# HKUST-Aerial-Robotics/Omni-swarm

Measured on AMD Instinct MI355X. Metric: keyframes/sec (4x fisheye 600x480) + p50 loop-match ms @ 100k-frame DB, higher is better.
Workload: dtype f16

## Files before the change

### omni-swarm_amd/csrc/config.h

```cpp
#pragma once
#include "common.h"

namespace omni {

enum CfgId {
    CFG_CONV_V1 = 0, CFG_RS_TRN, CFG_DET16, CFG_SP_SPARSE_DESC, CFG_SP_SPARSE_DA, CFG_SP_FUSED_CAND, CFG_SP_SPLIT_DB, CFG_SP_MASK_SKIP, CFG_SP_MASK_SKIP_SPLIT, CFG_SPLIT_FUSE1A, CFG_SPLIT_WINO,
    CFG_SPLIT_TRN, CFG_CONV_XCD, CFG_SP_PROFILE_MASK, CFG_PP_U8, CFG_PP_TRACE, CFG_PP_DBG, CFG_RS_TRACE, CFG_SPLIT_TRACE, CFG_SPLIT_DBG, CFG_WINO_TRACE, CFG_ROCTX,
    CFG_VLAD_BIG, CFG_VLAD_STEM_FUSE, CFG_VLAD_UNFUSED, CFG_VLAD_MFMA, CFG_VLAD_SBLOCK, CFG_VLAD_MBLOCK_PX, CFG_VLAD_MFMA_PX, CFG_VLAD_FC_MFMA, CFG_VLAD_MBLOCK_CPW,
    CFG_VLAD_SB_LDSPAD, CFG_VLAD_SB_PERSIST, CFG_VLAD_SB_TRACE, CFG_VLAD_SB_DBG, CFG_VLAD_MASK_SKIP,
    CFG_SCAN_ROWS_MIN, CFG_MQ_ROT, CFG_MQ_MIN, CFG_INDEX_MIRROR, CFG_INDEX_MIRROR_MIN_ROWS, CFG_INDEX_CERT_FAIL,
    CFG_GEOMETRY_THREADS, CFG_MESSAGE_THREADS, CFG_GEOMETRY_ASYNC, CFG_DETECTOR_ASYNC, CFG_PIPELINE_ONE_STREAM, CFG_PIPELINE_FIFO, CFG_PIPELINE_UNIT_PLAN,
    CFG_HW_QUEUES,
    CFG_RCCL_LIB,
    CFG_COUNT
};
enum CfgClass {
    CFG_VARIANT = 0,
    CFG_TUNING = 1,
    CFG_DEBUG = 2,
    CFG_TEST = 3,
    CFG_STRING = 4
};
struct CfgOption { const char* env; int def, lo, hi; int cls; const char* doc; };
extern const CfgOption kCfgOptions[CFG_COUNT];

struct Config {
    int v[CFG_COUNT];
    int operator[](CfgId i) const { return v[i]; }
};
int config_resolve(Config* out);
const Config& config_process();
int config_option_now(CfgId i);

}
```

### omni-swarm_amd/csrc/config.hip

```cpp
#include "config.h"

#include <atomic>
#include <cerrno>
#include <climits>
#include <cstdlib>

namespace omni {

const CfgOption kCfgOptions[CFG_COUNT] = {
    {"OMNI_CONV_V1", 0, 0, 3, CFG_VARIANT, "fp16 3x3 layers: 0 = production (conv1a fused into the ping-pong conv1b, register-stationary cin=128); 1 = generic kernel, 2 = persistent LDS-DMA kernel, "
                                           "3 = ping-pong without the conv1a fusion -- 1-3 exist only in the test build of the library (lib_test/)"},
    {"OMNI_RS_TRN", -1, -1, 1, CFG_VARIANT, "register-stationary kernel of the unpooled cin=128 fp16 layers: tile orientation, -1 = the one with fewer tiles, 0 = plain, 1 = transposed"},
    {"OMNI_DET16", 1, 0, 1, CFG_VARIANT, "detector head of the fp16 and OMNI_PREC_SPLIT paths on v_mfma_f32_32x32x16_f16 with split (hi, lo) operands (0: the exact-f32 MFMA kernel)"},
    {"OMNI_SP_SPARSE_DESC", 1, 0, 1, CFG_VARIANT, "convDb + descriptor norm only at the cells around the key points (0: dense descriptor map)"},
    {"OMNI_SP_SPARSE_DA", 1, 0, 1, CFG_VARIANT, "convDa only at those cells too (fp16 and OMNI_PREC_SPLIT; 0: dense convDa)"},
    {"OMNI_SP_FUSED_CAND", 1, 0, 1, CFG_VARIANT, "getKeyPoints' threshold inside the detector head's epilogue + window masks from the candidate list (0: sp_cand_kernel re-reads the heat map)"},
    {"OMNI_SP_SPLIT_DB", 1, 0, 1, CFG_VARIANT, "OMNI_PREC_SPLIT: convDb + descriptor norm at the key points' cells with split (hi, lo) operands on the fp16 matrix cores (0: exact-f32 MFMA convolution)"},
    {"OMNI_SP_MASK_SKIP", 1, 0, 1, CFG_VARIANT, "fp16: the tiles inside the constant region of the fisheye mask are left out of the tile walk (0: every tile)"},
    {"OMNI_SP_MASK_SKIP_SPLIT", 1, 0, 1, CFG_VARIANT, "the same for OMNI_PREC_SPLIT"},
    {"OMNI_SPLIT_FUSE1A", 1, 0, 1, CFG_VARIANT, "OMNI_PREC_SPLIT: conv1a built inside the conv1b kernel from the u8 image (0: separate exact-f32 conv1a pass)"},
    {"OMNI_SPLIT_WINO", 7, 0, 15, CFG_VARIANT, "OMNI_PREC_SPLIT: the cin = 64 layers as Winograd F(2x2,3x3) kernels with split operands (conv_wino.hip), bit 0 = conv1b (with the conv1a "
                                                "fusion), 1 = conv2a, 2 = conv2b, 3 = conv3a (off by default: same time as the direct kernel, profiles/r06g); 0: the direct kernels of conv_split.hip"},
    {"OMNI_SPLIT_TRN", -1, -1, 1, CFG_VARIANT, "OMNI_PREC_SPLIT cin=128 kernel: tile orientation, as OMNI_RS_TRN"},
    {"OMNI_CONV_XCD", 1, 0, 1, CFG_VARIANT, "persistent convolution kernels derive (cout group, tile walk) from an XCD-aware block id: the cout groups of a pixel tile and its neighbours "
                                           "share one L2 (0: plain blockIdx; process-wide, same results either way)"},
    {"OMNI_SP_PROFILE_MASK", 0, 0, 1, CFG_TUNING, "omni_sp_profile times the stages with the fisheye mask on (what the key-frame pipeline runs)"},
    {"OMNI_PP_U8", 1, 0, 1, CFG_VARIANT, "fp16 conv1a inside conv1b's kernel: matrix-core operands straight from the image bytes (0: through the 256-entry u8 -> (hi, lo) table in LDS)"},
    {"OMNI_PP_TRACE", 0, 0, 1, CFG_DEBUG, "s_memtime trace of the ping-pong conv kernel on stderr"},
    {"OMNI_PP_DBG", 0, 0, 255, CFG_DEBUG, "ping-pong conv kernel timing ablations (WRONG results)"},
    {"OMNI_RS_TRACE", 0, 0, 1, CFG_DEBUG, "s_memtime trace of the register-stationary kernel"},
    {"OMNI_SPLIT_TRACE", 0, 0, 1, CFG_DEBUG, "s_memtime trace of the split-precision kernel"},
    {"OMNI_SPLIT_DBG", 0, 0, 3, CFG_DEBUG, "split-precision kernel timing ablations: 1 = no stores, 2 = every DMA reads tile 0 (WRONG results)"},
    {"OMNI_WINO_TRACE", 0, 0, 1, CFG_DEBUG, "s_memtime trace of the Winograd split kernel"},
    {"OMNI_ROCTX", 0, 0, 1, CFG_DEBUG, "roctx ranges around upload / SuperPoint / MobileNetVLAD / post-processing / BF match / index add + search / exchange and the host loop's "
                                      "stages (rocprofv3 --marker-trace; the library is resolved by dlopen)"},
    {"OMNI_VLAD_BIG", 0, 0, 128, CFG_TUNING, "64 / 128: the 64- / 128-pixel tiles of the unfused block kernel (measured slower at 600x480)"},
    {"OMNI_VLAD_STEM_FUSE", 1, 0, 1, CFG_VARIANT, "stem + block 0 in one kernel (0: two kernels)"},
    {"OMNI_VLAD_UNFUSED", 0, 0, 1, CFG_VARIANT, "1: every block as expand / depthwise / project launches"},
    {"OMNI_VLAD_MFMA", 1, 0, 1, CFG_VARIANT, "late blocks' 1x1 convolutions on the matrix cores"},
    {"OMNI_VLAD_SBLOCK", 1, 0, 1, CFG_VARIANT, "fused split-fp16 block kernel (vlad_s.hip)"},
    {"OMNI_VLAD_MBLOCK_PX", 2048, 0, 1 << 24, CFG_TUNING, "fused matrix-core block kernel for blocks of at most this many input pixels per image (0 disables)"},
    {"OMNI_VLAD_MFMA_PX", 0, 0, 1 << 24, CFG_TUNING, "> 0: matrix-core 1x1 convolutions for blocks of at most this many input pixels per image (default 2048)"},
    {"OMNI_VLAD_FC_MFMA", 1, 0, 1, CFG_VARIANT, "the final FC on the matrix cores (0: VALU kernel)"},
    {"OMNI_VLAD_MBLOCK_CPW", 0, 0, 64, CFG_TUNING, "hidden-layer split of the matrix-core block kernel: chunks per workgroup (0 = no split; measured: does not pay)"},
    {"OMNI_VLAD_SB_LDSPAD", 0, 0, 160 * 1024, CFG_DEBUG, "extra LDS bytes per workgroup of the split block kernel (occupancy A/B)"},
    {"OMNI_VLAD_SB_PERSIST", 1, 0, 16, CFG_VARIANT, "split block kernel: 0 = one tile per workgroup, N >= 1 = N x (CUs x resident workgroups) persistent workgroups"},
    {"OMNI_VLAD_SB_TRACE", 0, 0, 1, CFG_DEBUG, "s_memtime trace of the split block kernel"},
    {"OMNI_VLAD_SB_DBG", 0, 0, 255, CFG_DEBUG, "split block kernel timing ablations (WRONG results)"},
    {"OMNI_VLAD_MASK_SKIP", 1, 0, 1, CFG_VARIANT, "fisheye-masked passes leave the tiles of the first blocks that lie in the constant region of the mask out of the tile walk "
                                                  "(bit-identical; 0: the dense pass)"},
    {"OMNI_SCAN_ROWS_MIN", 4, 1, 1 << 20, CFG_TUNING, "fp32 scan: from this many queries on, the rows-stationary kernel"},
    {"OMNI_MQ_ROT", 1, 0, 1, CFG_VARIANT, "matrix-core multi-query scan: rotated query fragments"},
    {"OMNI_MQ_MIN", 4, 0, 1 << 20, CFG_TUNING, "queries from which an fp16 shard is searched on the matrix cores (1 = always, 0 = never)"},
    {"OMNI_INDEX_MIRROR", 1, 0, 1, CFG_VARIANT, "fp32 index: fp16 mirror + certificate for batched searches (0: exact scans only)"},
    {"OMNI_INDEX_MIRROR_MIN_ROWS", 32768, 0, INT_MAX, CFG_TUNING, "the mirror is used from this many rows on"},
    {"OMNI_INDEX_CERT_FAIL", 0, 0, 1, CFG_TEST, "1: every certificate fails (exercises the exact fallback)"},
    {"OMNI_GEOMETRY_THREADS", -1, -1, 1024, CFG_TUNING, "threads of the geometric-verification pool (-1: min(16, cores / 2); 0: inline)"},
    {"OMNI_MESSAGE_THREADS", 3, 0, 64, CFG_TUNING, "helper threads that fill a unit's key-frame messages (key points, descriptors, lifted points: ~75 KB per image, first-touch page "
                                                  "faults included) next to the calling thread while the unit's detector step runs on the GPU (0: inline)"},
    {"OMNI_GEOMETRY_ASYNC", 1, 0, 1, CFG_VARIANT, "a micro-batch's geometry tasks run while the next unit is waited for (0: drained at once)"},
    {"OMNI_DETECTOR_ASYNC", 1, 0, 1, CFG_VARIANT, "a micro-batch's detector step (appends, searches) is enqueued and collected one unit later (0: the host waits for it on the spot)"},
    {"OMNI_PIPELINE_ONE_STREAM", 0, 0, 1, CFG_VARIANT, "a unit's MobileNetVLAD launches behind its SuperPoint launches on one stream (0: next to them on a second stream)"},
    {"OMNI_PIPELINE_FIFO", -1, -1, 2, CFG_VARIANT, "units in flight run oldest first: a unit's SuperPoint stream (1) / both its streams (2) start behind the convolution stack of the unit "
                                                   "enqueued before it; 0: the units' kernels take turns; -1: by measurement -- 1 for the fp32-class precisions, whose time is all "
                                                   "CU-filling convolutions (+2-4 %), and for an fp16 run() of no more units than lanes (all in flight at once: +13 % at 3 units), 0 for fp16 otherwise, whose small-grid "
                                                   "tails the next units' kernels fill (-5 % when chained)"},
    {"OMNI_PIPELINE_UNIT_PLAN", 1, 0, 2, CFG_VARIANT, "KeyframePipeline::run on host blocks, a run that is not a whole number of micro-batches: 1 = units of equal size (20 key frames = "
                                                       "7 + 7 + 6), 2 = the same behind half a unit, 0 = the blocks' own cut (8 + 8 + 4)"},
    {"OMNI_HW_QUEUES", 8, 0, 64, CFG_TUNING, "hardware queues asked of the HIP runtime when the library is loaded (GPU_MAX_HW_QUEUES, unless already set): the pipeline's five "
                                            "streams must not share one; 0 = the runtime's default of 4"},
    {"OMNI_RCCL_LIB", 0, 0, 0, CFG_STRING, "path of the RCCL library omni_shard dlopens (default: librccl.so next to torch, then the loader's search path)"},
};

static int parse_one(const CfgOption& o, int* out, bool* bad) {
    *out = o.def; *bad = false;
    if (o.cls == CFG_STRING) return 0;
    const char* e = getenv(o.env);
    if (!e || !e[0]) return 0;
    errno = 0;
    char* end = nullptr;
    const long v = strtol(e, &end, 10);
    if (errno || end == e || *end != '\0' || v < o.lo || v > o.hi) { *bad = true; return 0; }
    *out = (int)v;
    return 1;
}

int config_resolve(Config* out) {
    for (int i = 0; i < CFG_COUNT; ++i) {
        bool bad;
        parse_one(kCfgOptions[i], &out->v[i], &bad);
        OMNI_REQUIRE(!bad, OMNI_ERR_INVALID, "%s=%s: expected an integer in [%d, %d] (%s)", kCfgOptions[i].env, getenv(kCfgOptions[i].env), kCfgOptions[i].lo, kCfgOptions[i].hi,
                     kCfgOptions[i].doc);
    }
    return OMNI_OK;
}

static bool is_process_wide(int i) {
    switch (i) {
        case CFG_CONV_XCD: case CFG_INDEX_CERT_FAIL: case CFG_INDEX_MIRROR: case CFG_INDEX_MIRROR_MIN_ROWS: case CFG_MQ_ROT:
        case CFG_PP_DBG: case CFG_PP_TRACE: case CFG_RS_TRACE: case CFG_RS_TRN: case CFG_SCAN_ROWS_MIN: case CFG_SPLIT_DBG: case CFG_SPLIT_TRACE: case CFG_SPLIT_TRN: case CFG_WINO_TRACE: case CFG_ROCTX:
        case CFG_VLAD_BIG: case CFG_VLAD_SB_DBG: case CFG_VLAD_SB_LDSPAD: case CFG_VLAD_SB_TRACE:
            return true;
        default:
            return false;
    }
}
static std::atomic<bool> g_process_resolved{false};

int config_option_now(CfgId i) {
    int v; bool bad;
    parse_one(kCfgOptions[i], &v, &bad);
    return v;
}

const Config& config_process() {
    static const Config c = [] {
        g_process_resolved.store(true);
        Config q;
        for (int i = 0; i < CFG_COUNT; ++i) {
            bool bad;
            parse_one(kCfgOptions[i], &q.v[i], &bad);
            if (bad) fprintf(stderr, "libomni_hip: %s=%s ignored: expected an integer in [%d, %d]\n", kCfgOptions[i].env, getenv(kCfgOptions[i].env), kCfgOptions[i].lo, kCfgOptions[i].hi);
        }
        return q;
    }();
    return c;
}

}

extern "C" {

int omni_config_count(void) { return omni::CFG_COUNT; }
// ... 31 lines not shown
```

### omni-swarm_amd/csrc/vlad.hip

```cpp
#include "config.h"
#include "common.h"
#include "vlad_h.h"
#include "conv.h"

struct VladLayerDev { int kind, cin, cout, stride, hin, win, hout, wout; float* w; float* b; };

struct VladFusedBlock {
    int cin, hid, cout, stride, expand, res, hin, win, hout, wout;
    const float* bp;
    float* blob;
    float* mblob;
    void* hblob;
    void* sblob;
    int cop;
    const float *we_t, *be, *wd_t, *bd, *wp_t;
};

struct omni_vlad {
    omni_ctx* ctx = nullptr;
    omni::Config cfg;
    bool sblock = true;
    int prec = OMNI_PREC_F32;
    bool fused = false;
    bool mfma_late = true;
    int mblock_max_px = 0;
    int mfma_max_px = 2048;
    std::vector<VladFusedBlock> blocks;
    int W = 0, H = 0, max_batch = 0, K = 0, Dm = 0, out_dim = 0, hf = 0, wf = 0;
    std::vector<VladLayerDev> layers;
    float *assign_wT = nullptr, *assign_b = nullptr, *clusters = nullptr, *fc_w = nullptr, *fc_b = nullptr;
    float* mb_partial = nullptr; size_t mb_partial_bytes = 0; int mb_cpw = 1;
    float *fc_wp = nullptr, *fc_part = nullptr;
    bool fc_mfma = false;
    float *buf[3] = {nullptr, nullptr, nullptr};
    size_t buf_elems = 0;
    float *assign = nullptr, *vlad = nullptr, *out = nullptr;
    uint8_t* gray_stage = nullptr;
    omni::HostBuf hstage;
    struct MaskSkip {
        int ty0 = 0, ty1 = 0, tx0 = 0, tx1 = 0;
        int oy0 = 0, oy1 = 0, ox0 = 0, ox1 = 0;
        int oh = 0, ow = 0, oc = 0;
        float* buf = nullptr;
        void* vec = nullptr;
        double frac = 0.0;
    };
    std::vector<MaskSkip> mskip;
    bool mask_skip_ready = false;
    uint8_t* zero_gray = nullptr;
    std::mutex mu;
};

namespace omni {

__device__ __forceinline__ float relu6f(float v) { return fminf(fmaxf(v, 0.f), 6.f); }

__global__ void __launch_bounds__(256)
vlad_stem_kernel(const uint8_t* __restrict__ gray, int stride, int H, int W, int mask0, int mask1, int Ho, int Wo, int cout,
                 int cstride, const float* __restrict__ w , const float* __restrict__ bias, float* __restrict__ out) {
    const int b = blockIdx.y;
    const int p = blockIdx.x * 256 + threadIdx.x;
    if (p >= Ho * Wo) return;
    const int oy = p / Wo, ox = p - oy * Wo;
    const uint8_t* g = gray + (int64_t)b * stride * H;
    float v[9];
#pragma unroll
    for (int t = 0; t < 9; ++t) {
        const int y = oy * cstride - 1 + t / 3, x = ox * cstride - 1 + t % 3;
        float px = 0.f;
        if (y >= 0 && y < H && x >= 0 && x < W) {
            const float raw = (y >= mask0 && y < mask1) ? 0.f : (float)g[(int64_t)y * stride + x];
            px = (raw - 128.0f) / 128.0f;
        }
        v[t] = px;
    }
    float* o = out + ((int64_t)b * Ho * Wo + p) * cout;
    for (int c = 0; c < cout; ++c) {
        float acc = bias[c];
#pragma unroll
        for (int t = 0; t < 9; ++t) acc = fmaf(v[t], w[c * 9 + t], acc);
        o[c] = relu6f(acc);
    }
}

__global__ void __launch_bounds__(256)
// ... 880 lines not shown
    __shared__ float patch[PH * PW];
    __shared__ __attribute__((aligned(16))) float h[R * 16];
    __shared__ __attribute__((aligned(16))) float d[SB_TW * SB_TH * 16];
    __shared__ float s_ws[16 * 9], s_bs[16], s_wd[9 * 16], s_bd[16];
    const int tid = threadIdx.x, b = blockIdx.y;
    const int tiles_x = (Wo + SB_TW - 1) / SB_TW;
    const int oy0 = (blockIdx.x / tiles_x) * SB_TH, ox0 = (blockIdx.x % tiles_x) * SB_TW;
    const int sy0 = oy0 - 1, sx0 = ox0 - 1;
    const int iy0 = 2 * sy0 - 1, ix0 = 2 * sx0 - 1;
    if (tid < 144) { s_ws[tid] = ws[tid]; s_wd[tid] = wd_t[tid]; }
    if (tid < 16) { s_bs[tid] = bs[tid]; s_bd[tid] = bd[tid]; }
    const uint8_t* g = gray + (int64_t)b * stride * H;
    for (int i = tid; i < PH * PW; i += 256) {
        const int y = iy0 + i / PW, x = ix0 + i % PW;
        float px = 0.f;
        if (y >= 0 && y < H && x >= 0 && x < W) {
            const float raw = (y >= mask0 && y < mask1) ? 0.f : (float)g[(int64_t)y * stride + x];
            px = (raw - 128.0f) / 128.0f;
        }
        patch[i] = px;
    }
    __syncthreads();
    for (int i = tid; i < R * 4; i += 256) {
        const int r = i >> 2, c4 = (i & 3) * 4;
        const int ry = r / RW, rx = r - ry * RW;
        const int sy = sy0 + ry, sx = sx0 + rx;
        float4 res = make_float4(0.f, 0.f, 0.f, 0.f);
        if (sy >= 0 && sy < Ho && sx >= 0 && sx < Wo) {
            float v[9];
#pragma unroll
            for (int t = 0; t < 9; ++t) v[t] = patch[(2 * ry + t / 3) * PW + 2 * rx + t % 3];
            float rr[4];
#pragma unroll
            for (int j = 0; j < 4; ++j) {
                float acc = s_bs[c4 + j];
#pragma unroll
                for (int t = 0; t < 9; ++t) acc = fmaf(v[t], s_ws[(c4 + j) * 9 + t], acc);
                rr[j] = relu6f(acc);
            }
            res = make_float4(rr[0], rr[1], rr[2], rr[3]);
        }
        *reinterpret_cast<float4*>(h + r * 16 + c4) = res;
    }
    __syncthreads();
    for (int i = tid; i < SB_TW * SB_TH * 4; i += 256) {
        const int o = i >> 2, c4 = (i & 3) * 4;
        const int oy = o / SB_TW, ox = o - oy * SB_TW;
        float t[4];
#pragma unroll
        for (int j = 0; j < 4; ++j) t[j] = s_bd[c4 + j];
#pragma unroll
        for (int dy = 0; dy < 3; ++dy)
#pragma unroll
            for (int dx = 0; dx < 3; ++dx) {
                const float4 x = *reinterpret_cast<const float4*>(h + ((oy + dy) * RW + ox + dx) * 16 + c4);
                const float* wv = s_wd + (dy * 3 + dx) * 16 + c4;
                t[0] = fmaf(x.x, wv[0], t[0]); t[1] = fmaf(x.y, wv[1], t[1]); t[2] = fmaf(x.z, wv[2], t[2]); t[3] = fmaf(x.w, wv[3], t[3]);
            }
        *reinterpret_cast<float4*>(d + o * 16 + c4) = make_float4(relu6f(t[0]), relu6f(t[1]), relu6f(t[2]), relu6f(t[3]));
    }
    __syncthreads();
    {
        const int co = tid & 7, og = tid >> 3;
        float wp[16];
#pragma unroll
        for (int k = 0; k < 16; ++k) wp[k] = wp_t[k * 8 + co];
        const float bpv = bp[co];
#pragma unroll
        for (int i = 0; i < 4; ++i) {
            const int o = og + 32 * i;
            float acc = 0.f;
#pragma unroll
            for (int k4 = 0; k4 < 4; ++k4) {
                const float4 x = *reinterpret_cast<const float4*>(d + o * 16 + k4 * 4);
                acc = fmaf(x.x, wp[k4 * 4 + 0], acc); acc = fmaf(x.y, wp[k4 * 4 + 1], acc);
                acc = fmaf(x.z, wp[k4 * 4 + 2], acc); acc = fmaf(x.w, wp[k4 * 4 + 3], acc);
            }
            const int oy = oy0 + o / SB_TW, ox = ox0 + o % SB_TW;
            if (oy < Ho && ox < Wo) out[(((int64_t)b * Ho + oy) * Wo + ox) * 8 + co] = acc + bpv;
        }
    }
}

static int vlad_backbone_fused(omni_vlad* v, const uint8_t* gray_dev, int stride, int batch, int fisheye_mask, int skip_mode, const float** out_ptr) {
    hipStream_t st = v->ctx->stream;
    const int H = v->H, W = v->W;
    const float* in_over = nullptr;
    int m0, m1;
    omni_fisheye_mask_rows(H, fisheye_mask, &m0, &m1);
    const VladLayerDev& S = v->layers[0];
    int cur = 0, rc;
    size_t first = 0;
    const bool stem_fuse = v->cfg[omni::CFG_VLAD_STEM_FUSE] != 0;
    const VladFusedBlock* B0 = v->blocks.empty() ? nullptr : &v->blocks[0];
    if (stem_fuse && B0 && S.cout == 16 && S.stride == 2 && !B0->expand && !B0->res && B0->cin == 16 && B0->hid == 16 && B0->cout == 8 &&
        B0->stride == 1) {
        hipLaunchKernelGGL(vlad_stem_b0_kernel, dim3(cdiv(B0->wout, SB_TW) * cdiv(B0->hout, SB_TH), batch), dim3(256), 0, st, gray_dev, stride, H,
                           W, m0, m1, S.hout, S.wout, S.w, S.b, B0->wd_t, B0->bd, B0->wp_t, B0->bp, skip_mode ? v->mskip[0].buf : v->buf[1],
                           skip_mode == 2 ? v->mskip[0].ty0 : 0, skip_mode == 2 ? v->mskip[0].ty1 : 0, v->mskip.empty() ? 0 : v->mskip[0].tx0, v->mskip.empty() ? 0 : v->mskip[0].tx1);
        OMNI_LAUNCH_CHECK();
        cur = 1; first = 1;
        if (skip_mode) in_over = v->mskip[0].buf;
    } else {
        hipLaunchKernelGGL(vlad_stem4_kernel, dim3(cdiv(S.hout * S.wout * (S.cout / 4), 256), batch), dim3(256), 0, st, gray_dev, stride, H, W, m0,
                           m1, S.hout, S.wout, S.cout, S.stride, S.w, S.b, v->buf[0]);
        OMNI_LAUNCH_CHECK();
    }
    for (size_t bi = first; bi < v->blocks.size(); ++bi) {
        const VladFusedBlock& B = v->blocks[bi];
        const int64_t Pin = (int64_t)batch * B.hin * B.win, Pout = (int64_t)batch * B.hout * B.wout;
        const float* const in = in_over ? in_over : v->buf[cur];
        in_over = nullptr;
        if (v->prec == OMNI_PREC_F16 && B.hblob) {
            VladHBlockArgs ha;
            ha.in = in; ha.out = v->buf[(cur + 1) % 3]; ha.blob = B.hblob; ha.bp = B.bp;
            ha.Hi = B.hin; ha.Wi = B.win; ha.Ho = B.hout; ha.Wo = B.wout; ha.cin = B.cin; ha.hid = B.hid; ha.cout = B.cout; ha.res = B.res; ha.batch = batch;
            if ((rc = launch_vlad_hblock(st, ha, B.stride))) return rc;
            cur = (cur + 1) % 3;
            continue;
        }
        if (v->sblock && B.sblob) {
            VladSBlockArgs sa;
            const bool own = skip_mode && bi < v->mskip.size();
            sa.in = in; sa.out = own ? v->mskip[bi].buf : v->buf[(cur + 1) % 3]; sa.blob = B.sblob; sa.bp = B.bp;
            if (own && skip_mode == 2) { sa.sk_y0 = v->mskip[bi].ty0; sa.sk_y1 = v->mskip[bi].ty1; sa.sk_x0 = v->mskip[bi].tx0; sa.sk_w = v->mskip[bi].tx1 - v->mskip[bi].tx0; }
            sa.Hi = B.hin; sa.Wi = B.win; sa.Ho = B.hout; sa.Wo = B.wout; sa.cin = B.cin; sa.hid = B.hid; sa.cout = B.cout; sa.res = B.res; sa.batch = batch;
            sa.n_cu = v->ctx->prop.multiProcessorCount > 0 ? v->ctx->prop.multiProcessorCount : 256; sa.trace = nullptr; sa.dbg = 0;
            sa.persist = v->cfg[omni::CFG_VLAD_SB_PERSIST];
            if ((rc = launch_vlad_sblock(st, sa, B.stride))) return rc;
            if (own) in_over = v->mskip[bi].buf;
            else cur = (cur + 1) % 3;
            continue;
        }
        if (B.mblob && B.hin * B.win <= v->mblock_max_px) {
            VladMBlockArgs m;
            m.in = in; m.out = v->buf[(cur + 1) % 3]; m.blob = B.mblob; m.bp = B.bp;
            m.Hi = B.hin; m.Wi = B.win; m.Ho = B.hout; m.Wo = B.wout; m.cin = B.cin; m.hid = B.hid; m.cout = B.cout; m.cop = B.cop;
            m.stride = B.stride; m.res = B.res; m.batch = batch;
            const int n_chunks = (B.hid + 31) / 32, tiles = cdiv(B.wout, 8) * cdiv(B.hout, 8) * batch;
            m.cpw = v->mb_cpw > 0 ? v->mb_cpw : n_chunks; m.n_groups = cdiv(n_chunks, m.cpw);
            if ((size_t)tiles * m.n_groups * 64 * B.cop * 4 > v->mb_partial_bytes) { m.cpw = n_chunks; m.n_groups = 1; }
            m.partial = v->mb_partial;
            if ((rc = launch_vlad_mblock(st, m))) return rc;
            cur = (cur + 1) % 3;
            continue;
        }
        if (B.expand && B.cin % 8 == 0 && B.hid % 8 == 0 && B.hin * B.win <= v->mfma_max_px && v->mfma_late) {
            const int e = (cur + 1) % 3, d = (cur + 2) % 3;
            if ((rc = vlad_pw_mfma(st, in, Pin, B.cin, B.hid, B.we_t, B.be, nullptr, 1, v->buf[e]))) return rc;
            const int64_t total = Pout * (B.hid / 4);
            hipLaunchKernelGGL(vlad_dw_kernel, dim3((unsigned)cdiv64(total, 256)), dim3(256), 0, st, v->buf[e], B.hin, B.win, B.hid, B.hout, B.wout,
                               B.stride, B.wd_t, B.bd, v->buf[d], total);
            OMNI_LAUNCH_CHECK();
            if ((rc = vlad_pw_mfma(st, v->buf[d], Pout, B.hid, B.cout, B.wp_t, B.bp, B.res ? in : nullptr, 0, v->buf[e]))) return rc;
            cur = e;
            continue;
        }
        VladBlockArgs a;
        a.in = in; a.out = v->buf[(cur + 1) % 3];
        a.blob = B.blob; a.bp = B.bp;
        a.Hi = B.hin; a.Wi = B.win; a.Ho = B.hout; a.Wo = B.wout; a.hid = B.hid; a.cout = B.cout; a.stride = B.stride;
        a.expand = B.expand; a.res = B.res; a.batch = batch;
        if ((rc = vlad_block(st, B.cin, a))) return rc;
        cur = (cur + 1) % 3;
    }
    *out_ptr = in_over ? in_over : v->buf[cur];
    return OMNI_OK;
}

static int vlad_calibrate_mask_skip(omni_vlad* v) {
    hipStream_t st = v->ctx->stream;
    if (!v->zero_gray) {
        OMNI_HIP_TRY(hipMalloc((void**)&v->zero_gray, (size_t)v->W * v->H));
        OMNI_HIP_TRY(hipMemsetAsync(v->zero_gray, 0, (size_t)v->W * v->H, st));
    }
    const float* unused;
    int rc;
    if ((rc = vlad_backbone_fused(v, v->zero_gray, v->W, 1, 1, 1, &unused))) return rc;
    for (const omni_vlad::MaskSkip& k : v->mskip) {
        const int pix = k.oc * 4;
        const int64_t row = (int64_t)k.ow * pix, img = row * k.oh;
        if ((rc = conv_read_pixel_bytes(st, k.buf, row, 0, pix, (k.oy0 + k.oy1) / 2, (k.ox0 + k.ox1) / 2, k.vec))) return rc;
        if ((rc = conv_fill_rect_bytes(st, k.buf, v->max_batch, img, row, 0, pix, k.oy0, k.oy1, k.ox0, k.ox1, k.vec))) return rc;
// ... 372 lines not shown
```

### omni-swarm_amd/csrc/vlad_s.hip

```cpp
#include "config.h"
#include "common.h"
#include "vlad_h.h"

namespace omni {

typedef _Float16 sh8 __attribute__((ext_vector_type(8)));
typedef _Float16 sh4 __attribute__((ext_vector_type(4)));
typedef _Float16 sh2 __attribute__((ext_vector_type(2)));
typedef float sf16 __attribute__((ext_vector_type(16)));
typedef float sf2 __attribute__((ext_vector_type(2)));
typedef float sf4 __attribute__((ext_vector_type(4)));

#define SB_CH 48
#define SB_HS 208
#define SB_DS 112
#define SB_WD (10 * SB_CH)

__device__ __forceinline__ int sb_div(int n, unsigned m) { return m ? (int)__umulhi((unsigned)n, m) : n; }

template <int STRIDE, int CIN, int NT>
struct SBlockCfg {
    static constexpr int S1 = (2 * CIN + 2 + 15) / 16, S2 = (CIN + 15) / 16;
    static constexpr int XS = S1 * 32 + 16;
    static constexpr int TH = STRIDE == 1 ? 8 : 4, OPX = 8 * TH, NTN = OPX / 32;
// ... 7 lines not shown
#ifndef SB_WPE_SMALL
#define SB_WPE_SMALL 2
#endif
template <int STRIDE, int CIN, int NT>
__global__ void __launch_bounds__((SBlockCfg<STRIDE, CIN, NT>::THREADS), (CIN > 32 ? 1 : (CIN <= 16 ? SB_WPE_SMALL : 2)))
vlad_sblock_kernel(VladSBlockArgs a) {
    using C = SBlockCfg<STRIDE, CIN, NT>;
    constexpr int S1 = C::S1, S2 = C::S2, XS = C::XS, TH = C::TH, OPX = C::OPX, RWX = C::RWX, R = C::R, CB = C::CB, MQ = C::MQ, NW = C::NW, RT = C::RT, XP = C::XP;
    extern __shared__ __attribute__((aligned(16))) char smem[];
    const int n_chunks = a.hid / SB_CH;
    char* xin = smem;
    char* dhi = smem + R * XS;
    char* dlo = dhi + OPX * SB_DS;
    char* h = dlo + OPX * SB_DS;
    float* wdl = reinterpret_cast<float*>(h + R * SB_HS);
    const int tid = threadIdx.x, lane = tid & 63, wave = __builtin_amdgcn_readfirstlane(tid >> 6);
    const int n = lane & 31, kk = lane >> 5;
    const int tiles_x = (a.Wo + 7) >> 3, tiles_y = (a.Ho + TH - 1) / TH, tiles_img = tiles_x * tiles_y;
    const char* blob = reinterpret_cast<const char*>(a.blob);
    const char* frag = blob + (size_t)n_chunks * SB_WD * 4;

    sh8 we1[S1][2], we2[S2][2];
    auto load_we = [&](int c) {
        const char* cb = frag + (int64_t)c * CB + lane * 16;
#pragma unroll
        for (int ks = 0; ks < S1; ++ks)
#pragma unroll
            for (int m = 0; m < 2; ++m) we1[ks][m] = *reinterpret_cast<const sh8*>(cb + (ks * 2 + m) * 1024);
#pragma unroll
        for (int ks = 0; ks < S2; ++ks)
#pragma unroll
            for (int m = 0; m < 2; ++m) we2[ks][m] = *reinterpret_cast<const sh8*>(cb + ((S1 + ks) * 2 + m) * 1024);
    };
    load_we(0);
    {
        const sf4* ws = reinterpret_cast<const sf4*>(blob);
        for (int e = tid; e < n_chunks * (SB_WD / 4); e += C::THREADS) reinterpret_cast<sf4*>(wdl)[e] = ws[e];
    }
    const int pair = tid % 24, blk = tid / 24;
    const int nt = STRIDE == 1 ? (wave & 1) : 0;
    const int mt0 = STRIDE == 1 ? (wave >> 1) : wave;
    constexpr int MSTEP = STRIDE == 1 ? 2 : NW;
    const bool pwave = mt0 < NT;
    sf4 pbias[MQ][4];
#pragma unroll
    for (int q = 0; q < MQ; ++q)
#pragma unroll
        for (int g = 0; g < 4; ++g) {
            const int ch = (mt0 + MSTEP * q) * 32 + 8 * g + 4 * kk;
            const sf4 z = {0.f, 0.f, 0.f, 0.f};
            pbias[q][g] = ch < a.cout ? *reinterpret_cast<const sf4*>(a.bp + ch) : z;
        }

    auto tile_origin = [&](int tile, int& tb, int& toy, int& tox) {
        tb = sb_div(tile, a.m_img);
        const int ttr = tile - tb * tiles_img, tty = sb_div(ttr, a.m_tx);
        toy = tty * TH; tox = (ttr - tty * tiles_x) * 8;
    };
    const int act_total = a.walk.act * a.batch;
    auto full_tile = [&](int t) -> int {
        if (a.walk.y1 <= a.walk.y0) return t;
        const int tb = sb_div(t, a.m_act);
        return tb * tiles_img + tile_walk_index(a.walk, tiles_x, t - tb * a.walk.act);
    };
    const int xhf = tid & 1;
    sf4 xpre[XP][CIN / 8];
    bool xin_img[XP];
    auto fetch_x = [&](int tile) {
        int tb, toy, tox;
        tile_origin(tile, tb, toy, tox);
#pragma unroll
        for (int ps = 0; ps < XP; ++ps) {
            const int xr = (tid >> 1) + ps * (C::THREADS / 2), xry = xr / RWX, xrx = xr - xry * RWX;
            const int gy = toy * STRIDE - 1 + xry, gx = tox * STRIDE - 1 + xrx;
            xin_img[ps] = xr < R && gy >= 0 && gy < a.Hi && gx >= 0 && gx < a.Wi;
            const unsigned off = (unsigned)((tb * a.Hi + gy) * a.Wi + gx) * CIN + xhf * (CIN / 2);
#pragma unroll
            for (int q = 0; q < CIN / 8; ++q) {
                const sf4 z = {0.f, 0.f, 0.f, 0.f};
                xpre[ps][q] = xin_img[ps] ? *reinterpret_cast<const sf4*>(a.in + off + q * 4) : z;
            }
        }
    };
    sf16 acc[MQ];
    sf4 resv[MQ][4];
    unsigned out_off = 0;
    bool out_ok = false;
    auto out_pixel = [&](int tile, unsigned& off_out, unsigned& off_res) {
        int tb, toy, tox;
        tile_origin(tile, tb, toy, tox);
        const int o = nt * 32 + n, oy = toy + (o >> 3), ox = tox + (o & 7);
        off_out = (unsigned)((tb * a.Ho + oy) * a.Wo + ox) * (unsigned)a.cout;
        off_res = (unsigned)((tb * a.Hi + oy) * a.Wi + ox) * (unsigned)CIN;
        return pwave && oy < a.Ho && ox < a.Wo;
    };
    auto fetch_res = [&](bool ok, unsigned off_res) {
        if (!a.res) return;
#pragma unroll
        for (int q = 0; q < MQ; ++q)
#pragma unroll
            for (int g = 0; g < 4; ++g) {
                const int ch = (mt0 + MSTEP * q) * 32 + 8 * g + 4 * kk;
                const sf4 z = {0.f, 0.f, 0.f, 0.f};
                resv[q][g] = (ok && ch < a.cout) ? *reinterpret_cast<const sf4*>(a.in + off_res + ch) : z;
            }
    };
    auto store_out = [&]() {
        if (!out_ok || (a.dbg & 1)) return;
#pragma unroll
        for (int q = 0; q < MQ; ++q)
#pragma unroll
            for (int g = 0; g < 4; ++g) {
                const int ch = (mt0 + MSTEP * q) * 32 + 8 * g + 4 * kk;
                if (ch >= a.cout) continue;
                sf4 v = pbias[q][g];
#pragma unroll
                for (int j = 0; j < 4; ++j) v[j] += acc[q][4 * g + j];
                if (a.res) v += resv[q][g];
                *reinterpret_cast<sf4*>(a.out + out_off + ch) = v;
            }
    };

    auto expand = [&]() {
#pragma unroll
      for (int rt = 0; rt < (RT + NW - 1) / NW; ++rt) {
        const int rw = wave + rt * NW;
        if (rw >= RT) break;
        const char* xb = xin + (rw * 32 + n) * XS + kk * 16;
        sf16 e0, e1;
#pragma unroll
        for (int r = 0; r < 16; ++r) { e0[r] = 0.f; e1[r] = 0.f; }
#pragma unroll
        for (int ks = 0; ks < S1; ++ks) {
            const sh8 xb8 = *reinterpret_cast<const sh8*>(xb + ks * 32);
            e0 = __builtin_amdgcn_mfma_f32_32x32x16_f16(we1[ks][0], xb8, e0, 0, 0, 0);
            e1 = __builtin_amdgcn_mfma_f32_32x32x16_f16(we1[ks][1], xb8, e1, 0, 0, 0);
        }
#pragma unroll
        for (int ks = 0; ks < S2; ++ks) {
            const sh8 xb8 = *reinterpret_cast<const sh8*>(xb + ks * 32);
            e0 = __builtin_amdgcn_mfma_f32_32x32x16_f16(we2[ks][0], xb8, e0, 0, 0, 0);
            e1 = __builtin_amdgcn_mfma_f32_32x32x16_f16(we2[ks][1], xb8, e1, 0, 0, 0);
        }
        if (rw * 32 + n < R) {
            char* hp = h + (rw * 32 + n) * SB_HS + kk * 16;
#pragma unroll
            for (int g = 0; g < 4; ++g) {
                sf4 v;
#pragma unroll
                for (int j = 0; j < 4; ++j) v[j] = __builtin_amdgcn_fmed3f(e0[4 * g + j], 0.f, 6.f);
                *reinterpret_cast<sf4*>(hp + g * 32) = v;
            }
#pragma unroll
            for (int g = 0; g < 2; ++g) {
                sf4 v;
#pragma unroll
                for (int j = 0; j < 4; ++j) v[j] = __builtin_amdgcn_fmed3f(e1[4 * g + j], 0.f, 6.f);
                *reinterpret_cast<sf4*>(hp + 128 + g * 32) = v;
            }
        }
      }
    };

    if ((int)blockIdx.x < act_total) fetch_x(full_tile(blockIdx.x));
#define TR(k) do { if (trw) a.trace[wave * 16 + (k)] = __builtin_amdgcn_s_memtime(); } while (0)
    for (int t = blockIdx.x; t < act_total; t += gridDim.x) {
        const int tile = full_tile(t);
        const bool trw = a.trace && blockIdx.x == 0 && (tid & 63) == 0 && t == (int)blockIdx.x + 2 * (int)gridDim.x;
        TR(8);
#pragma unroll
        for (int ps = 0; ps < XP; ++ps) {
            const int xr = (tid >> 1) + ps * (C::THREADS / 2);
            if (xr < R) {
                char* row = xin + xr * XS;
#pragma unroll
                for (int q = 0; q < CIN / 8; ++q) {
                    const sf4 v = xpre[ps][q];
                    const sh4 hi = __builtin_convertvector(v, sh4);
                    const sh4 lo = __builtin_convertvector(v - __builtin_convertvector(hi, sf4), sh4);
                    *reinterpret_cast<sh4*>(row + (xhf * (CIN / 2) + q * 4) * 2) = hi;
                    *reinterpret_cast<sh4*>(row + CIN * 2 + (xhf * (CIN / 2) + q * 4) * 2) = lo;
                }
                sh8 t = {0, 0, 0, 0, 0, 0, 0, 0};
                if (xhf == 0 && xin_img[ps]) { t[0] = (_Float16)1.f; t[1] = (_Float16)1.f; }
                *reinterpret_cast<sh8*>(row + CIN * 4 + xhf * 16) = t;
            }
        }
        store_out();
        {
            unsigned off_res;
            out_ok = out_pixel(tile, out_off, off_res);
            fetch_res(out_ok, off_res);
        }
        if (t + (int)gridDim.x < act_total && !(a.dbg & 2)) fetch_x(full_tile(t + gridDim.x));
#pragma unroll
        for (int p = 0; p < MQ; ++p)
#pragma unroll
            for (int r = 0; r < 16; ++r) acc[p][r] = 0.f;

        __syncthreads();
        TR(0);
// ... 76 lines not shown
                expand();
                __syncthreads();
            }
            TR(6);
        }
        TR(7);
    }
#undef TR
    store_out();
}

static inline uint16_t sb_f2h(float v) { const __half hv = __float2half_rn(v); uint16_t u; memcpy(&u, &hv, 2); return u; }
static inline float sb_h2f(uint16_t u) { __half hv; memcpy(&hv, &u, 2); return __half2float(hv); }
static inline float sb_hi(float v) { return sb_h2f(sb_f2h(v)); }
static inline float sb_lo(float v) { return v - sb_hi(v); }

#define SB_SHAPES(X) X(2, 8, 1) X(1, 8, 1) X(1, 16, 1) X(2, 16, 1) X(1, 24, 1) X(1, 32, 1) X(2, 32, 2) X(1, 56, 2) X(1, 56, 4)

bool vlad_sblock_supported(int cin, int hid, int cout, int stride) {
    if (hid < SB_CH || hid % SB_CH || cout % 4 || cout < 4) return false;
    const int nt0 = (cout + 31) / 32, nt = nt0 == 3 ? 4 : nt0;
#define X(S, CI, N) if (stride == S && cin == CI && nt == N) return true;
    SB_SHAPES(X)
#undef X
    return false;
}

static inline int sb_nt(int cout) { const int nt0 = (cout + 31) / 32; return nt0 == 3 ? 4 : nt0; }

size_t vlad_sblock_blob_bytes(int cin, int hid, int cout) {
    const int S1 = (2 * cin + 2 + 15) / 16, S2 = (cin + 15) / 16, NT = sb_nt(cout);
    return (size_t)(hid / SB_CH) * (SB_WD * 4 + (S1 + S2) * 2048 + NT * 6144);
}

void vlad_sblock_pack(int cin, int hid, int cout, const float* we, const float* be, const float* wd, const float* bd, const float* wp, void* out) {
    const int S1 = (2 * cin + 2 + 15) / 16, S2 = (cin + 15) / 16, NT = sb_nt(cout), CB = (S1 + S2) * 2048 + NT * 6144;
    const int n_chunks = hid / SB_CH;
    memset(out, 0, vlad_sblock_blob_bytes(cin, hid, cout));
    float* wdo = reinterpret_cast<float*>(out);
    for (int ch = 0; ch < hid; ++ch) {
        float* q = wdo + (size_t)(ch / SB_CH) * SB_WD + ch % SB_CH;
        for (int t = 0; t < 9; ++t) q[t * SB_CH] = wd[(size_t)ch * 9 + t];
        q[9 * SB_CH] = bd[ch];
    }
    char* frag = reinterpret_cast<char*>(out) + (size_t)n_chunks * SB_WD * 4;
    for (int c = 0; c < n_chunks; ++c) {
        char* cb = frag + (size_t)c * CB;
        for (int pass = 0; pass < 2; ++pass)
            for (int ks = 0; ks < (pass ? S2 : S1); ++ks)
                for (int m = 0; m < 2; ++m)
                    for (int l = 0; l < 64; ++l)
                        for (int e = 0; e < 8; ++e) {
                            const int row = m * 32 + (l & 31), k = ks * 16 + (l >> 5) * 8 + e;
                            float v = 0.f;
                            if (row < SB_CH) {
                                const int ch = c * SB_CH + row;
                                if (!pass) {
                                    if (k < cin) v = sb_hi(we[(size_t)ch * cin + k]);
                                    else if (k < 2 * cin) v = sb_hi(we[(size_t)ch * cin + k - cin]);
                                    else if (k == 2 * cin) v = sb_hi(be[ch]);
                                    else if (k == 2 * cin + 1) v = sb_lo(be[ch]);
                                } else if (k < cin) v = sb_lo(we[(size_t)ch * cin + k]);
                            }
                            reinterpret_cast<uint16_t*>(cb + (((pass ? S1 : 0) + ks) * 2 + m) * 1024)[l * 8 + e] = sb_f2h(v);
                        }
        for (int m = 0; m < NT; ++m)
            for (int ks = 0; ks < 3; ++ks)
                for (int part = 0; part < 2; ++part)
                    for (int l = 0; l < 64; ++l)
                        for (int e = 0; e < 8; ++e) {
                            const int co = m * 32 + (l & 31), hc = c * SB_CH + ks * 16 + (l >> 5) * 8 + e;
                            float v = 0.f;
                            if (co < cout) v = part ? sb_lo(wp[(size_t)co * hid + hc]) : sb_hi(wp[(size_t)co * hid + hc]);
                            reinterpret_cast<uint16_t*>(cb + (S1 + S2) * 2048 + ((m * 3 + ks) * 2 + part) * 1024)[l * 8 + e] = sb_f2h(v);
                        }
    }
}

template <int STRIDE, int CIN, int NT>
static int launch_sb(hipStream_t st, const VladSBlockArgs& a) {
    using C = SBlockCfg<STRIDE, CIN, NT>;
    static const size_t pad = (size_t)config_process()[CFG_VLAD_SB_LDSPAD];
    const size_t smem = C::smem(a.hid) + pad;
    OMNI_REQUIRE(smem <= 160 * 1024, OMNI_ERR_CAPACITY, "vlad_sblock: %zu B of LDS for hid=%d", smem, a.hid);
    auto kfn = vlad_sblock_kernel<STRIDE, CIN, NT>;
    static DynSmemState attr;
    OMNI_HIP_TRY(ensure_dyn_smem(attr, (const void*)kfn, smem));
    const int tiles_x = cdiv(a.Wo, 8), tiles_y = cdiv(a.Ho, C::TH);
    VladSBlockArgs at = a;
    if (int rc = tile_walk_plan(at.walk, "vlad_sblock", tiles_x, tiles_y, a.sk_y0, a.sk_y1, a.sk_x0, a.sk_x0 + a.sk_w)) return rc;
    const int tiles = at.walk.act * a.batch;
    OMNI_REQUIRE((int64_t)a.batch * a.Hi * a.Wi * a.cin < (1ll << 31) && (int64_t)a.batch * a.Ho * a.Wo * a.cout < (1ll << 31) && tiles < (1 << 20),
                 OMNI_ERR_CAPACITY, "vlad_sblock: tensor beyond 32-bit element offsets");
    static int per_cu_cached = 0;
    static size_t per_cu_smem = 0;
    if (!per_cu_cached || per_cu_smem != smem) {
        int nb = 0;
        OMNI_HIP_TRY(hipOccupancyMaxActiveBlocksPerMultiprocessor(&nb, (const void*)kfn, C::THREADS, smem));
        per_cu_cached = nb < 1 ? 1 : nb;
        per_cu_smem = smem;
    }
    const int per_cu = per_cu_cached;
    const int persist = a.persist;
    const int64_t cap = (int64_t)a.n_cu * per_cu * (persist > 0 ? persist : 1);
    const int grid = (!persist || tiles < cap) ? tiles : (int)cap;
    static const bool want_trace = config_process()[CFG_VLAD_SB_TRACE] != 0;
    static unsigned long long* trace_dev = nullptr;
    at.trace = nullptr;
    static const int dbg = config_process()[CFG_VLAD_SB_DBG];
    at.dbg = dbg;
    at.m_img = tile_walk_magic(tiles_x * tiles_y);
    at.m_tx = tile_walk_magic(tiles_x);
    at.m_act = tile_walk_magic(at.walk.act);
    if (want_trace) {
        if (!trace_dev) OMNI_HIP_TRY(hipMalloc((void**)&trace_dev, 8 * 16 * 8));
        OMNI_HIP_TRY(hipMemsetAsync(trace_dev, 0, 8 * 16 * 8, st));
        at.trace = trace_dev;
    }
    hipLaunchKernelGGL(kfn, dim3(grid), dim3(C::THREADS), smem, st, at);
    OMNI_LAUNCH_CHECK();
    if (want_trace) {
        unsigned long long hbuf[8 * 16];
        OMNI_HIP_TRY(hipMemcpyAsync(hbuf, trace_dev, sizeof(hbuf), hipMemcpyDeviceToHost, st));
        OMNI_HIP_TRY(hipStreamSynchronize(st));
        static int launches = 0;
        if (launches++ == 8)
            for (int w = 0; w < C::THREADS / 64; ++w) {
                const unsigned long long* t = hbuf + w * 16;
                if (!t[8]) continue;
                fprintf(stderr, "sb trace s%d cin%d grid %d wave %d (last chunk): x->lds+store+bar %llu expand %llu bar %llu | dw %llu bar %llu proj %llu | tile %llu\n",
                        STRIDE, CIN, grid, w, t[0] - t[8], t[1] - t[0], t[2] - t[1], t[3] - t[2], t[4] - t[3], t[5] - t[4], t[7] - t[8]);
            }
    }
    return OMNI_OK;
}

int launch_vlad_sblock(hipStream_t st, const VladSBlockArgs& a, int stride) {
    const int nt = sb_nt(a.cout);
#define X(S, CI, N) if (stride == S && a.cin == CI && nt == N) return launch_sb<S, CI, N>(st, a);
    SB_SHAPES(X)
#undef X
    set_error("vlad_sblock: no instantiation for cin=%d cout=%d stride=%d", a.cin, a.cout, stride);
    return OMNI_ERR_INVALID;
}

}
```

Measured before the change: 2754.

## Run stem + block 0 as persistent tile-walking workgroups with prefetched patches

Adds a persistent variant of the fused stem + block-0 VLAD kernel, enabled by default. Workgroups walk the mask-skipped tile list, prefetch the next tile's image bytes into registers while the current tile is computed, and keep the block-0 projection weights in registers across tiles. This removes per-tile launch and weight-load overhead and overlaps global reads with compute. It also makes the split-block kernel's residual path compile-time dead for stride 2. The cost is extra register pressure and a grid capped at CUs × occupancy, which may leave load imbalance on a small stage.

```diff
diff --git a/omni-swarm_amd/csrc/config.h b/omni-swarm_amd/csrc/config.h
--- a/omni-swarm_amd/csrc/config.h
+++ b/omni-swarm_amd/csrc/config.h
@@ -7,7 +7,7 @@
     CFG_CONV_V1 = 0, CFG_RS_TRN, CFG_DET16, CFG_SP_SPARSE_DESC, CFG_SP_SPARSE_DA, CFG_SP_FUSED_CAND, CFG_SP_SPLIT_DB, CFG_SP_MASK_SKIP, CFG_SP_MASK_SKIP_SPLIT, CFG_SPLIT_FUSE1A, CFG_SPLIT_WINO,
     CFG_SPLIT_TRN, CFG_CONV_XCD, CFG_SP_PROFILE_MASK, CFG_PP_U8, CFG_PP_TRACE, CFG_PP_DBG, CFG_RS_TRACE, CFG_SPLIT_TRACE, CFG_SPLIT_DBG, CFG_WINO_TRACE, CFG_ROCTX,
     CFG_VLAD_BIG, CFG_VLAD_STEM_FUSE, CFG_VLAD_UNFUSED, CFG_VLAD_MFMA, CFG_VLAD_SBLOCK, CFG_VLAD_MBLOCK_PX, CFG_VLAD_MFMA_PX, CFG_VLAD_FC_MFMA, CFG_VLAD_MBLOCK_CPW,
-    CFG_VLAD_SB_LDSPAD, CFG_VLAD_SB_PERSIST, CFG_VLAD_SB_TRACE, CFG_VLAD_SB_DBG, CFG_VLAD_MASK_SKIP,
+    CFG_VLAD_SB_LDSPAD, CFG_VLAD_SB_PERSIST, CFG_VLAD_SB_TRACE, CFG_VLAD_SB_DBG, CFG_VLAD_MASK_SKIP, CFG_VLAD_STEM_PERSIST,
     CFG_SCAN_ROWS_MIN, CFG_MQ_ROT, CFG_MQ_MIN, CFG_INDEX_MIRROR, CFG_INDEX_MIRROR_MIN_ROWS, CFG_INDEX_CERT_FAIL,
     CFG_GEOMETRY_THREADS, CFG_MESSAGE_THREADS, CFG_GEOMETRY_ASYNC, CFG_DETECTOR_ASYNC, CFG_PIPELINE_ONE_STREAM, CFG_PIPELINE_FIFO, CFG_PIPELINE_UNIT_PLAN,
     CFG_HW_QUEUES,
diff --git a/omni-swarm_amd/csrc/config.hip b/omni-swarm_amd/csrc/config.hip
--- a/omni-swarm_amd/csrc/config.hip
+++ b/omni-swarm_amd/csrc/config.hip
@@ -49,6 +49,7 @@
     {"OMNI_VLAD_SB_DBG", 0, 0, 255, CFG_DEBUG, "split block kernel timing ablations (WRONG results)"},
     {"OMNI_VLAD_MASK_SKIP", 1, 0, 1, CFG_VARIANT, "fisheye-masked passes leave the tiles of the first blocks that lie in the constant region of the mask out of the tile walk "
                                                   "(bit-identical; 0: the dense pass)"},
+    {"OMNI_VLAD_STEM_PERSIST", 1, 0, 1, CFG_TUNING, "stem + block 0 as persistent workgroups that walk the tiles, weights in scalar registers (0: one workgroup per tile; bit-identical)"},
     {"OMNI_SCAN_ROWS_MIN", 4, 1, 1 << 20, CFG_TUNING, "fp32 scan: from this many queries on, the rows-stationary kernel"},
     {"OMNI_MQ_ROT", 1, 0, 1, CFG_VARIANT, "matrix-core multi-query scan: rotated query fragments"},
     {"OMNI_MQ_MIN", 4, 0, 1 << 20, CFG_TUNING, "queries from which an fp16 shard is searched on the matrix cores (1 = always, 0 = never)"},
diff --git a/omni-swarm_amd/csrc/vlad.hip b/omni-swarm_amd/csrc/vlad.hip
--- a/omni-swarm_amd/csrc/vlad.hip
+++ b/omni-swarm_amd/csrc/vlad.hip
@@ -1,6 +1,7 @@
 #include "config.h"
 #include "common.h"
 #include "vlad_h.h"
+#include "vlad_stem_tile.h"
 #include "conv.h"
 
 struct VladLayerDev { int kind, cin, cout, stride, hin, win, hout, wout; float* w; float* b; };
@@ -1047,6 +1048,155 @@
     }
 }
 
+struct VladStemB0Args {
+    int stride, H, W, mask0, mask1, Ho, Wo;
+    int batch, tiles_x;
+    TileWalk walk;
+    unsigned m_act;
+};
+__global__ void __launch_bounds__(VST_THREADS, 4)
+vlad_stem_b0_persist_kernel(const uint8_t* __restrict__ gray, const float* __restrict__ ws , const float* __restrict__ bs,
+                            const float* __restrict__ wd_t , const float* __restrict__ bd, const float* __restrict__ wp_t ,
+                            const float* __restrict__ bp, float* __restrict__ out , VladStemB0Args a) {
+    typedef float f4 __attribute__((ext_vector_type(4)));
+    __shared__ float patch[VST_P];
+    __shared__ __attribute__((aligned(16))) f4 h4[4 * VST_R];
+    __shared__ __attribute__((aligned(16))) f4 d4[4 * VST_O];
+    __shared__ __attribute__((aligned(16))) float s_wd[10 * 16];
+    const int tid = threadIdx.x, lane = tid & 63, wave = __builtin_amdgcn_readfirstlane(tid >> 6);
+    const int total = a.walk.act * a.batch;
+    int p_rc[VST_NP], r_tap[VST_NR], r_rc[VST_NR], o_tap, o_px;
+#pragma unroll
+    for (int k = 0; k < VST_NP; ++k) {
+        int py, px;
+        p_rc[k] = vlad_stem_patch_rc(tid + VST_THREADS * k, py, px) ? (py << 8 | px) : -1;
+    }
+#pragma unroll
+    for (int k = 0; k < VST_NR; ++k) {
+        int ry, rx;
+        r_rc[k] = vlad_stem_region_rc(lane + 64 * k, ry, rx, r_tap[k]) ? (ry << 8 | rx) : -1;
+    }
+    {
+        int oy, ox;
+        vlad_stem_out_rc(lane, oy, ox, o_tap);
+        o_px = oy * VST_TW + ox;
+    }
+    int pre[VST_NP];
+    auto fetch = [&](int t) {
+        const StemTile s = vlad_stem_tile(a.walk, a.tiles_x, a.m_act, t);
+        const uint8_t* g = gray + (int64_t)s.b * a.stride * a.H;
+#pragma unroll
+        for (int k = 0; k < VST_NP; ++k) {
+            const int y = s.iy0 + (p_rc[k] >> 8), x = s.ix0 + (p_rc[k] & 255);
+            int v = -1;
+            if (p_rc[k] >= 0 && y >= 0 && y < a.H && x >= 0 && x < a.W) v = (y >= a.mask0 && y < a.mask1) ? 0 : (int)g[(int64_t)y * a.stride + x];
+            pre[k] = v;
+        }
+    };
+    const int c4 = wave * 4;
+    if (tid < 10 * 16) s_wd[tid] = tid < 9 * 16 ? wd_t[tid] : bd[tid - 9 * 16];
+    const int co = tid & 7, og = tid >> 3;
+    float wp[16];
+#pragma unroll
+    for (int k = 0; k < 16; ++k) wp[k] = wp_t[k * 8 + co];
+    const float bpv = bp[co];
+    if ((int)blockIdx.x < total) fetch(blockIdx.x);
+    for (int t = blockIdx.x; t < total; t += gridDim.x) {
+        const StemTile s = vlad_stem_tile(a.walk, a.tiles_x, a.m_act, t);
+#pragma unroll
+        for (int k = 0; k < VST_NP; ++k)
+            if (p_rc[k] >= 0) patch[tid + VST_THREADS * k] = pre[k] < 0 ? 0.f : ((float)pre[k] - 128.0f) / 128.0f;
+        if (t + (int)gridDim.x < total) fetch(t + gridDim.x);
+        __syncthreads();
+#pragma unroll
+        for (int k = 0; k < VST_NR; ++k) {
+            if (r_rc[k] < 0) continue;
+            const int sy = s.sy0 + (r_rc[k] >> 8), sx = s.sx0 + (r_rc[k] & 255);
+            f4 res = {0.f, 0.f, 0.f, 0.f};
+            if (sy >= 0 && sy < a.Ho && sx >= 0 && sx < a.Wo) {
+                float v[9];
+#pragma unroll
+                for (int q = 0; q < 9; ++q) v[q] = patch[r_tap[k] + (q / 3) * VST_PW + q % 3];
+#pragma unroll
+                for (int j = 0; j < 4; ++j) {
+                    float acc = bs[c4 + j];
+#pragma unroll
+                    for (int q = 0; q < 9; ++q) acc = fmaf(v[q], ws[(c4 + j) * 9 + q], acc);
+                    res[j] = relu6f(acc);
+                }
+            }
+            h4[wave * VST_R + lane + 64 * k] = res;
+        }
+        __syncthreads();
+        {
+            f4 wdv[10];
+#pragma unroll
+            for (int q = 0; q < 10; ++q) wdv[q] = *reinterpret_cast<const f4*>(s_wd + q * 16 + c4);
+            const f4* hp = h4 + wave * VST_R + o_tap;
+            f4 x[4][3];
+#pragma unroll
+            for (int r = 0; r < 4; ++r)
+#pragma unroll
+                for (int dx = 0; dx < 3; ++dx) x[r][dx] = hp[r * VST_RW + dx];
+#pragma unroll
+            for (int k = 0; k < VST_NO; ++k) {
+                f4 acc = wdv[9];
+#pragma unroll
+                for (int dy = 0; dy < 3; ++dy)
+#pragma unroll
+                    for (int dx = 0; dx < 3; ++dx)
+#pragma unroll
+                        for (int j = 0; j < 4; ++j) acc[j] = fmaf(x[k + dy][dx][j], wdv[dy * 3 + dx][j], acc[j]);
+#pragma unroll
+                for (int j = 0; j < 4; ++j) acc[j] = relu6f(acc[j]);
+                d4[wave * VST_O + o_px + VST_TW * k] = acc;
+            }
+        }
+        __syncthreads();
+#pragma unroll
+        for (int i = 0; i < VST_O / 32; ++i) {
+            const int o = og + 32 * i;
+            float acc = 0.f;
+#pragma unroll
+            for (int k4 = 0; k4 < 4; ++k4) {
+                const f4 x = d4[k4 * VST_O + o];
+#pragma unroll
+                for (int kk = 0; kk < 4; ++kk) acc = fmaf(x[kk], wp[k4 * 4 + kk], acc);
+            }
+            const int oy = s.oy0 + o / VST_TW, ox = s.ox0 + o % VST_TW;
+            if (oy < a.Ho && ox < a.Wo) out[(((int64_t)s.b * a.Ho + oy) * a.Wo + ox) * 8 + co] = acc + bpv;
+        }
+    }
+}
+static_assert(VST_TW == SB_TW && VST_TH == SB_TH, "the mask-skip plan and both stem + block 0 kernels share one tile shape");
+
+static int launch_vlad_stem_b0_persist(omni_vlad* v, const uint8_t* gray_dev, int stride, int batch, int m0, int m1, float* out, int ty0, int ty1,
+                                       int tx0, int tx1) {
+    const VladLayerDev& S = v->layers[0];
+    const VladFusedBlock& B0 = v->blocks[0];
+    VladStemB0Args a;
+    a.stride = stride; a.H = v->H; a.W = v->W; a.mask0 = m0; a.mask1 = m1; a.Ho = S.hout; a.Wo = S.wout;
+    a.batch = batch;
+    a.tiles_x = cdiv(B0.wout, VST_TW);
+    if (int rc = tile_walk_plan(a.walk, "vlad_stem_b0", a.tiles_x, cdiv(B0.hout, VST_TH), ty0, ty1, tx0, tx1)) return rc;
+    const int64_t tiles = (int64_t)a.walk.act * batch;
+    OMNI_REQUIRE(tiles * a.walk.act < (1ll << 32), OMNI_ERR_CAPACITY, "vlad_stem_b0: %lld tiles: too many for the multiply-high division",
+                 (long long)tiles);
+    a.m_act = tile_walk_magic(a.walk.act);
+    static int per_cu = 0;
+    if (!per_cu) {
+        int nb = 0;
+        OMNI_HIP_TRY(hipOccupancyMaxActiveBlocksPerMultiprocessor(&nb, (const void*)vlad_stem_b0_persist_kernel, VST_THREADS, 0));
+        per_cu = nb < 1 ? 1 : nb;
+    }
+    const int n_cu = v->ctx->prop.multiProcessorCount > 0 ? v->ctx->prop.multiProcessorCount : 256;
+    const int64_t cap = (int64_t)n_cu * per_cu;
+    hipLaunchKernelGGL(vlad_stem_b0_persist_kernel, dim3((unsigned)(tiles < cap ? tiles : cap)), dim3(VST_THREADS), 0, v->ctx->stream, gray_dev, S.w, S.b,
+                       B0.wd_t, B0.bd, B0.wp_t, B0.bp, out, a);
+    OMNI_LAUNCH_CHECK();
+    return OMNI_OK;
+}
+
 static int vlad_backbone_fused(omni_vlad* v, const uint8_t* gray_dev, int stride, int batch, int fisheye_mask, int skip_mode, const float** out_ptr) {
     hipStream_t st = v->ctx->stream;
     const int H = v->H, W = v->W;
@@ -1060,10 +1210,17 @@
     const VladFusedBlock* B0 = v->blocks.empty() ? nullptr : &v->blocks[0];
     if (stem_fuse && B0 && S.cout == 16 && S.stride == 2 && !B0->expand && !B0->res && B0->cin == 16 && B0->hid == 16 && B0->cout == 8 &&
         B0->stride == 1) {
-        hipLaunchKernelGGL(vlad_stem_b0_kernel, dim3(cdiv(B0->wout, SB_TW) * cdiv(B0->hout, SB_TH), batch), dim3(256), 0, st, gray_dev, stride, H,
-                           W, m0, m1, S.hout, S.wout, S.w, S.b, B0->wd_t, B0->bd, B0->wp_t, B0->bp, skip_mode ? v->mskip[0].buf : v->buf[1],
-                           skip_mode == 2 ? v->mskip[0].ty0 : 0, skip_mode == 2 ? v->mskip[0].ty1 : 0, v->mskip.empty() ? 0 : v->mskip[0].tx0, v->mskip.empty() ? 0 : v->mskip[0].tx1);
-        OMNI_LAUNCH_CHECK();
+        float* const o0 = skip_mode ? v->mskip[0].buf : v->buf[1];
+        if (v->cfg[omni::CFG_VLAD_STEM_PERSIST]) {
+            const bool sk = skip_mode == 2;
+            if ((rc = launch_vlad_stem_b0_persist(v, gray_dev, stride, batch, m0, m1, o0, sk ? v->mskip[0].ty0 : 0, sk ? v->mskip[0].ty1 : 0,
+                                                  sk ? v->mskip[0].tx0 : 0, sk ? v->mskip[0].tx1 : 0))) return rc;
+        } else {
+            hipLaunchKernelGGL(vlad_stem_b0_kernel, dim3(cdiv(B0->wout, SB_TW) * cdiv(B0->hout, SB_TH), batch), dim3(256), 0, st, gray_dev, stride, H,
+                               W, m0, m1, S.hout, S.wout, S.w, S.b, B0->wd_t, B0->bd, B0->wp_t, B0->bp, o0,
+                               skip_mode == 2 ? v->mskip[0].ty0 : 0, skip_mode == 2 ? v->mskip[0].ty1 : 0, v->mskip.empty() ? 0 : v->mskip[0].tx0, v->mskip.empty() ? 0 : v->mskip[0].tx1);
+            OMNI_LAUNCH_CHECK();
+        }
         cur = 1; first = 1;
         if (skip_mode) in_over = v->mskip[0].buf;
     } else {
diff --git a/omni-swarm_amd/csrc/vlad_s.hip b/omni-swarm_amd/csrc/vlad_s.hip
--- a/omni-swarm_amd/csrc/vlad_s.hip
+++ b/omni-swarm_amd/csrc/vlad_s.hip
@@ -113,6 +113,7 @@
             }
         }
     };
+    const bool has_res = STRIDE == 1 && a.res;
     sf16 acc[MQ];
     sf4 resv[MQ][4];
     unsigned out_off = 0;
@@ -126,7 +127,7 @@
         return pwave && oy < a.Ho && ox < a.Wo;
     };
     auto fetch_res = [&](bool ok, unsigned off_res) {
-        if (!a.res) return;
+        if (!has_res) return;
 #pragma unroll
         for (int q = 0; q < MQ; ++q)
 #pragma unroll
@@ -147,7 +148,7 @@
                 sf4 v = pbias[q][g];
 #pragma unroll
                 for (int j = 0; j < 4; ++j) v[j] += acc[q][4 * g + j];
-                if (a.res) v += resv[q][g];
+                if (has_res) v += resv[q][g];
                 *reinterpret_cast<sf4*>(a.out + out_off + ch) = v;
             }
     };
@@ -390,6 +391,7 @@
     using C = SBlockCfg<STRIDE, CIN, NT>;
     static const size_t pad = (size_t)config_process()[CFG_VLAD_SB_LDSPAD];
     const size_t smem = C::smem(a.hid) + pad;
+    OMNI_REQUIRE(STRIDE == 1 || !a.res, OMNI_ERR_INVALID, "vlad_sblock: a residual needs stride 1");
     OMNI_REQUIRE(smem <= 160 * 1024, OMNI_ERR_CAPACITY, "vlad_sblock: %zu B of LDS for hid=%d", smem, a.hid);
     auto kfn = vlad_sblock_kernel<STRIDE, CIN, NT>;
     static DynSmemState attr;
diff --git a/omni-swarm_amd/csrc/vlad_stem_tile.h b/omni-swarm_amd/csrc/vlad_stem_tile.h
--- /dev/null
+++ b/omni-swarm_amd/csrc/vlad_stem_tile.h
@@ -0,0 +1,47 @@
+#pragma once
+#include "tile_walk.h"
+
+namespace omni {
+
+constexpr int VST_TW = 16, VST_TH = 8, VST_O = VST_TW * VST_TH;
+constexpr int VST_RW = VST_TW + 2, VST_RH = VST_TH + 2, VST_R = VST_RW * VST_RH;
+constexpr int VST_PW = 2 * VST_RW + 1, VST_PH = 2 * VST_RH + 1, VST_P = VST_PW * VST_PH;
+constexpr int VST_THREADS = 256;
+constexpr int VST_NP = (VST_P + VST_THREADS - 1) / VST_THREADS;
+constexpr int VST_NR = (VST_R + 63) / 64;
+constexpr int VST_NO = VST_O / 64;
+static_assert(VST_NO == 2 && VST_TW * (VST_TH / 2) == 64, "a wave's lanes are the tile's columns x its row pairs");
+
+struct StemTile {
+    int b;
+    int oy0, ox0;
+    int sy0, sx0;
+    int iy0, ix0;
+};
+
+TW_HD StemTile vlad_stem_tile(const TileWalk& k, int tiles_x, uint32_t m_act, int t) {
+    StemTile s;
+    s.b = tile_walk_div(t, m_act);
+    int ty, tx;
+    tile_walk_rc(k, tiles_x, t - s.b * k.act, ty, tx);
+    s.oy0 = ty * VST_TH; s.ox0 = tx * VST_TW;
+    s.sy0 = s.oy0 - 1; s.sx0 = s.ox0 - 1;
+    s.iy0 = 2 * s.sy0 - 1; s.ix0 = 2 * s.sx0 - 1;
+    return s;
+}
+
+TW_HD bool vlad_stem_patch_rc(int i, int& py, int& px) {
+    py = i / VST_PW; px = i - py * VST_PW;
+    return i < VST_P;
+}
+TW_HD bool vlad_stem_region_rc(int r, int& ry, int& rx, int& tap0) {
+    ry = r / VST_RW; rx = r - ry * VST_RW;
+    tap0 = 2 * ry * VST_PW + 2 * rx;
+    return r < VST_R;
+}
+TW_HD void vlad_stem_out_rc(int lane, int& oy, int& ox, int& tap0) {
+    oy = 2 * (lane / VST_TW); ox = lane - (lane / VST_TW) * VST_TW;
+    tap0 = oy * VST_RW + ox;
+}
+
+}
```

After: 2772 (median of 6 runs). No clear change (+0.7%).
